# AIS-Bonn/stillleben

Measured on AMD Instinct MI355X. Metric: scenes/sec (settle + 640x480 6-ch GT render), 20-obj YCB-like, higher is better.
Workload: dtype f32; 1 GPU; C2: 20 of 21 procedural YCB-like objects (8k verts/16k tris, 1024^2 texture each) per scene; per step and GPU 32768 scenes are staged (random stack), settled (100 frames x 4 substeps), framed (camera, light, shadow matrix) and rendered at 640x480 (rgb, coord+depth, class, instance, normals; shadows on, SSAO on) -- all four stages inside the timed region; render_chunk=512, objects=20, settle_streams=1, render_streams=2, pair_contact_budget=0, parallelism=1 GPU

## Files before the change

### stillleben_amd/csrc/slhip_render.hip

```cpp
#include <algorithm>
#include <cmath>
#include <cstring>
#include <vector>
#include <type_traits>
#include "slhip_common.h"
#include "slhip_cubemap.h"
#include "slhip_raster_walk.h"

#ifndef SLHIP_RENDER_WAVES
#define SLHIP_RENDER_WAVES 0
#endif
#ifndef SLHIP_SHADE_WAVES
#define SLHIP_SHADE_WAVES 0
#endif
#ifndef SLHIP_SSAO_WAVES
#define SLHIP_SSAO_WAVES 0
#endif
#if SLHIP_RENDER_WAVES > 0
#define SLHIP_LIGHT_KERNEL __attribute__((amdgpu_waves_per_eu(1, SLHIP_RENDER_WAVES)))
#else
#define SLHIP_LIGHT_KERNEL
#endif
#if SLHIP_RENDER_WAVES > 0
#define SLHIP_SHADOW_RASTER_KERNEL SLHIP_LIGHT_KERNEL
#else
#define SLHIP_SHADOW_RASTER_KERNEL __attribute__((amdgpu_waves_per_eu(6)))
#endif
#if SLHIP_SSAO_WAVES > 0
#define SLHIP_SSAO_KERNEL __attribute__((amdgpu_waves_per_eu(1, SLHIP_SSAO_WAVES)))
#else
#define SLHIP_SSAO_KERNEL
#endif
#if SLHIP_SHADE_WAVES > 0
#define SLHIP_SHADE_KERNEL __attribute__((amdgpu_waves_per_eu(1, SLHIP_SHADE_WAVES)))
#else
#define SLHIP_SHADE_KERNEL
#endif
namespace {

static_assert(sizeof(slhip_draw) == 432, "slhip_draw layout");
static_assert(sizeof(slhip_scene) == 480, "slhip_scene layout");
static_assert(sizeof(slhip_chunk) == 16, "slhip_chunk layout");

constexpr float kInvalid = 3000.0f;
constexpr float kPi = 3.141592653589793f;
constexpr unsigned long long kVisEmpty = ~0ull;
constexpr int kSmallArea = 256;

__device__ __forceinline__ float dot3(const float* a, const float* b)
{
    float d = a[0] * b[0];
    d = fmaf(a[1], b[1], d);
    d = fmaf(a[2], b[2], d);
    return d;
}

__device__ __forceinline__ void mv4(const float* __restrict__ M, const float* v, float* o)
{
#pragma unroll
    for (int r = 0; r < 4; ++r) {
// ... 540 lines not shown
            float b[3];
#pragma unroll
            for (int k = 0; k < 3; ++k)
                b[k] = fmaf(bs[2], bary[6 + k], fmaf(bs[1], bary[3 + k], bs[0] * bary[k]));
            if (peel) {
                const float cz = interp(b, camz[0], camz[1], camz[2]);
                if (cz - 0.00001f <= peel[4 * ((size_t)py * W + px) + 3]) return;
            }
            if (pool_tex) {
                const float u = interp(b, uv[0], uv[2], uv[4]);
                const float v = interp(b, uv[1], uv[3], uv[5]);
                float bx[3], by[3];
                bary_at(t, bary, bary + 3, bary + 6, px + 1, py, bx);
                bary_at(t, bary, bary + 3, bary + 6, px, py + 1, by);
                float tc[4];
                tex_sample(pool_tex, tex, tex_w, tex_h, tex_sampler, u, v, interp(bx, uv[0], uv[2], uv[4]) - u, interp(bx, uv[1], uv[3], uv[5]) - v,
                           interp(by, uv[0], uv[2], uv[4]) - u, interp(by, uv[1], uv[3], uv[5]) - v, tc);
                if (base_alpha * tc[3] < alpha_cutoff) return;
            }
        }
        atomicMin(slot, key);
    }
};

#ifndef SLHIP_SHADOW_WINDOW
#define SLHIP_SHADOW_WINDOW 64
#endif
#ifndef SLHIP_SHADOW_WINDOW_PITCH
#define SLHIP_SHADOW_WINDOW_PITCH SLHIP_SHADOW_WINDOW
#endif
struct ShadowTarget {
    unsigned* sm;
    int W;
    unsigned* win;
    int wx0, wy0;
    unsigned wnx, wny;
    __device__ __forceinline__ void emit(const Setup& t, int px, int py, const float* l) const
    {
        const float z = interp(l, t.z[0], t.z[1], t.z[2]);
        if (!(z >= 0.0f && z <= 1.0f)) return;
        const unsigned bits = __float_as_uint(z);
#if SLHIP_SHADOW_WINDOW
        const unsigned ux = (unsigned)(px - wx0), uy = (unsigned)(py - wy0);
        if (ux < wnx && uy < wny) {
            atomicMin(win + uy * SLHIP_SHADOW_WINDOW_PITCH + ux, bits);
            return;
        }
#endif
        unsigned* slot = sm + (size_t)py * W + px;
        atomicMin(slot, bits);
    }
};

struct QItem {
    unsigned draw;
    unsigned tri_sub;
    unsigned scene_aux;
    unsigned tile;
};

template <class I, class Target>
__device__ __forceinline__ void raster_bbox_as(const Setup& t, const Target& tgt)
{
    slhip_raster::Walk<I> w;
    w.start(t.X, t.Y, t.flipped, t.bias, t.xmin, t.ymin);
    const float fa = (float)(I)t.area2;
    const int bw = t.xmax - t.xmin + 1, n = bw * (t.ymax - t.ymin + 1);
    int px = t.xmin, py = t.ymin;
    for (int k = 0; k < n; ++k) {
        if (w.inside()) {
            float l[3];
            l[0] = (float)w.numerator(0) / fa;
            l[1] = (float)w.numerator(1) / fa;
            l[2] = (float)w.numerator(2) / fa;
            tgt.emit(t, px, py, l);
        }
        if (px == t.xmax) {
            px = t.xmin; ++py;
            w.next_row();
        } else {
            ++px;
            w.step_x();
        }
    }
}

template <class Target>
__device__ __forceinline__ void raster_bbox(const Setup& t, const Target& tgt, int wide)
{
    if (!wide && __all(t.narrow)) {
        raster_bbox_as<int>(t, tgt);
    } else {
        const int bw = t.xmax - t.xmin + 1, n = bw * (t.ymax - t.ymin + 1);
        int px = t.xmin, py = t.ymin;
        for (int k = 0; k < n; ++k) {
            float l[3];
            if (coverage_as<long long>(t, px, py, l)) tgt.emit(t, px, py, l);
            if (px == t.xmax) { px = t.xmin; ++py; } else ++px;
        }
    }
}

template <class Target>
__device__ __forceinline__ void raster_or_enqueue(const Setup& t, const Target& tgt, unsigned* queue,
                                                  unsigned capacity, unsigned draw, unsigned tri_sub,
                                                  unsigned scene_aux, int small_area, int wide = 0)
{
    const int bw = t.xmax - t.xmin + 1, bh = t.ymax - t.ymin + 1;
    bool in_place = bw * bh <= small_area;
    if (!in_place) {
        const int tx0 = t.xmin >> 3, tx1 = t.xmax >> 3, ty0 = t.ymin >> 3, ty1 = t.ymax >> 3;
        const unsigned n = (unsigned)((tx1 - tx0 + 1) * (ty1 - ty0 + 1));
        const unsigned base = atomicAdd(queue, n);
        if (base + n <= capacity) {
            QItem* items = reinterpret_cast<QItem*>(queue + 4);
            unsigned k = base;
            for (int ty = ty0; ty <= ty1; ++ty)
                for (int tx = tx0; tx <= tx1; ++tx) {
                    QItem it;
                    it.draw = draw; it.tri_sub = tri_sub; it.scene_aux = scene_aux;
                    it.tile = (unsigned)tx | ((unsigned)ty << 16);
                    items[k++] = it;
                }
        } else {
            QItem* items = reinterpret_cast<QItem*>(queue + 4);
            for (unsigned k = base; k < min(base + n, capacity); ++k) {
                QItem it;
                it.draw = 0xFFFFFFFFu; it.tri_sub = 0; it.scene_aux = 0; it.tile = 0;
                items[k] = it;
            }
            in_place = true;
        }
    }
    if (in_place) raster_bbox(t, tgt, wide);
}

template <bool kAttr>
__device__ __forceinline__ void raster_chunk(unsigned chunk, const slhip_mesh_pool& pool, const slhip_scene* __restrict__ scenes,
                                             const slhip_draw* __restrict__ draws,
                                             const slhip_chunk* __restrict__ chunks, int W, int H,
                                             const float* __restrict__ depth_peel,
                                             unsigned long long* __restrict__ vis, unsigned* queue,
                                             unsigned capacity, const float4* __restrict__ clipbuf,
                                             const uint4* __restrict__ screen, int small_area, int wide)
{
    const slhip_chunk ch = chunks[chunk];
    if (threadIdx.x >= ch.count) return;
    const slhip_scene* sc = scenes + ch.scene;
    const slhip_draw* dr = draws + ch.draw;
    const bool alpha_test = (dr->flags & SLHIP_DRAW_ALPHA_TEST) && (dr->flags & SLHIP_DRAW_HAS_BASE_TEX);
    if ((alpha_test || depth_peel != nullptr) != kAttr) return;
    const unsigned tri = ch.first_tri + threadIdx.x;
    const unsigned* ip = pool.d_idx + dr->idx_base + 3 * (size_t)tri;
    const unsigned vi[3] = {ip[0], ip[1], ip[2]};
    const size_t P = (size_t)W * H;
    MainTarget tgt;
    tgt.vis = vis + (size_t)ch.scene * P;
    tgt.W = W;
    tgt.prim = dr->prim_base + tri;
    tgt.need_attr = kAttr;
    tgt.peel = nullptr;
    tgt.pool_tex = nullptr;

    if constexpr (!kAttr) {
        tgt.camz = nullptr; tgt.uv = nullptr; tgt.bary = nullptr;
        const uint4 s0 = screen[dr->clip_base + vi[0]], s1 = screen[dr->clip_base + vi[1]], s2 = screen[dr->clip_base + vi[2]];
        if (screen_all_inside(s0, s1, s2)) {
            Setup t;
            if (setup_from_screen(s0, s1, s2, W, H, t)) raster_or_enqueue(t, tgt, queue, capacity, ch.draw, tri, ch.scene, small_area, wide);
            return;
        }
        ClipVert cv[3];
#pragma unroll
        for (int k = 0; k < 3; ++k) {
            const float4 c4 = clipbuf[dr->clip_base + vi[k]];
            cv[k].clip[0] = c4.x; cv[k].clip[1] = c4.y; cv[k].clip[2] = c4.z; cv[k].clip[3] = c4.w;
            cv[k].bary[0] = cv[k].bary[1] = cv[k].bary[2] = 0.0f;
        }
        ClipVert poly[4];
        const int n = clip_near(cv, poly);
#pragma unroll
        for (int sub = 0; sub < 2; ++sub) {
            if (sub >= n - 2) break;
            Setup t;
            if (!setup_tri(poly[0].clip, poly[sub + 1].clip, poly[sub + 2].clip, W, H, t)) continue;
// ... 24 lines not shown
            for (int k = 0; k < 3; ++k) {
                const float2 uv = reinterpret_cast<const float2*>(pool.d_uv)[dr->vtx_base + vi[k]];
                uvs[2 * k] = uv.x; uvs[2 * k + 1] = uv.y;
            }
            tgt.pool_tex = pool.d_tex; tgt.tex = dr->tex_offset;
            tgt.tex_w = (int)dr->tex_w; tgt.tex_h = (int)dr->tex_h;
            tgt.tex_sampler = dr->tex_sampler[0];
        }
        tgt.camz = camz;
        tgt.uv = uvs;
        tgt.base_alpha = dr->base_color[3];
        tgt.alpha_cutoff = dr->alpha_cutoff;
#pragma unroll
        for (int sub = 0; sub < 2; ++sub) {
            if (sub >= n - 2) break;
            Setup t;
            if (!setup_tri(poly[0].clip, poly[sub + 1].clip, poly[sub + 2].clip, W, H, t)) continue;
            float bary[9];
#pragma unroll
            for (int k = 0; k < 3; ++k) {
                bary[k] = poly[0].bary[k];
                bary[3 + k] = poly[sub + 1].bary[k];
                bary[6 + k] = poly[sub + 2].bary[k];
            }
            tgt.bary = bary;
            for (int py = t.ymin; py <= t.ymax; ++py)
                for (int px = t.xmin; px <= t.xmax; ++px) {
                    float l[3];
                    if (coverage(t, px, py, l)) tgt.emit(t, px, py, l);
                }
        }
    }
}

template <bool kAttr>
__global__ __launch_bounds__(256) SLHIP_LIGHT_KERNEL void k_raster(slhip_mesh_pool pool, const slhip_scene* __restrict__ scenes,
                                                const slhip_draw* __restrict__ draws,
                                                const slhip_chunk* __restrict__ chunks, unsigned n_chunks, int W, int H,
                                                const float* __restrict__ depth_peel,
                                                unsigned long long* __restrict__ vis, unsigned* queue,
                                                unsigned capacity, const float4* __restrict__ clipbuf,
                                                const uint4* __restrict__ screen, int small_area, int wide)
{
    for (unsigned c = blockIdx.x; c < n_chunks; c += gridDim.x)
        raster_chunk<kAttr>(c, pool, scenes, draws, chunks, W, H, depth_peel, vis, queue, capacity, clipbuf, screen, small_area, wide);
}

__global__ __launch_bounds__(256) SLHIP_LIGHT_KERNEL void k_large(slhip_mesh_pool pool, const slhip_scene* __restrict__ scenes,
                                               const slhip_draw* __restrict__ draws, int W, int H,
                                               unsigned long long* __restrict__ vis,
                                               const unsigned* __restrict__ queue, unsigned capacity,
                                               const float4* __restrict__ clipbuf, const uint4* __restrict__ screen)
{
    const unsigned count = min(queue[0], capacity);
    const QItem* items = reinterpret_cast<const QItem*>(queue + 4);
    const unsigned lane = threadIdx.x & 63;
    const unsigned wave = (blockIdx.x * blockDim.x + threadIdx.x) >> 6;
    const unsigned n_waves = (gridDim.x * blockDim.x) >> 6;
    const unsigned per = (count + n_waves - 1) / n_waves;
    const unsigned i0 = wave * per, i1 = min(i0 + per, count);
    unsigned p_draw = 0xFFFFFFFFu, p_tri = 0u, p_scene = 0u, prim = 0u;
    bool ok = false;
    Setup t;
    for (unsigned i = i0; i < i1; ++i) {
        const QItem it = items[i];
        if (it.draw == 0xFFFFFFFFu) continue;
        if (it.draw != p_draw || it.tri_sub != p_tri || it.scene_aux != p_scene) {
            p_draw = it.draw; p_tri = it.tri_sub; p_scene = it.scene_aux;
            ok = false;
            const slhip_draw* dr = draws + it.draw;
            const unsigned tri = it.tri_sub & 0x7FFFFFFFu;
            const int sub = (int)(it.tri_sub >> 31);
            const unsigned* ip = pool.d_idx + dr->idx_base + 3 * (size_t)tri;
            ClipVert cv[3];
            const uint4 s0 = screen[dr->clip_base + ip[0]], s1 = screen[dr->clip_base + ip[1]], s2 = screen[dr->clip_base + ip[2]];
            const bool cached = screen_all_inside(s0, s1, s2);
            if (cached && (sub != 0 || !setup_from_screen(s0, s1, s2, W, H, t))) continue;
            if (!cached) {
#pragma unroll
                for (int k = 0; k < 3; ++k) {
                    const float4 c4 = clipbuf[dr->clip_base + ip[k]];
                    cv[k].clip[0] = c4.x; cv[k].clip[1] = c4.y; cv[k].clip[2] = c4.z; cv[k].clip[3] = c4.w;
                    cv[k].bary[0] = cv[k].bary[1] = cv[k].bary[2] = 0.0f;
                }
                ClipVert poly[4];
                const int n = clip_near(cv, poly);
                if (sub > n - 3) continue;
                const ClipVert& pb = sub == 0 ? poly[1] : poly[2];
                const ClipVert& pc = sub == 0 ? poly[2] : poly[3];
                if (!setup_tri(poly[0].clip, pb.clip, pc.clip, W, H, t)) continue;
            }
            prim = dr->prim_base + tri;
            ok = true;
        }
        if (!ok) continue;
        const int px = (int)((it.tile & 0xFFFFu) << 3) + (int)(lane & 7);
        const int py = (int)((it.tile >> 16) << 3) + (int)(lane >> 3);
        if (px < t.xmin || px > t.xmax || py < t.ymin || py > t.ymax) continue;
        float l[3];
        if (!coverage(t, px, py, l)) continue;
        MainTarget tgt;
        tgt.vis = vis + (size_t)it.scene_aux * W * H;
        tgt.peel = nullptr;
        tgt.W = W;
        tgt.prim = prim;
        tgt.need_attr = false;
        tgt.pool_tex = nullptr;
        tgt.emit(t, px, py, l);
    }
}

__device__ __forceinline__ void shadow_clip(const slhip_mesh_pool& pool, const float* T, unsigned v, float* clip)
{
    const float4 p = reinterpret_cast<const float4*>(pool.d_pos)[v];
    const float pos[4] = {p.x, p.y, p.z, 1.0f};
#pragma unroll
    for (int r = 0; r < 4; ++r) {
        float a = fmaf(T[4 * r + 0], pos[0], 0.0f);
        a = fmaf(T[4 * r + 1], pos[1], a);
        a = fmaf(T[4 * r + 2], pos[2], a);
        a = fmaf(T[4 * r + 3], pos[3], a);
        clip[r] = a;
    }
}

template <bool kMax>
__device__ __forceinline__ int wave_minmax(int v)
{
    constexpr int ident = kMax ? (int)0x80000000 : 0x7fffffff;
#define SLHIP_DPP_STEP(ctrl, rows)                                                       \
    {                                                                                    \
        const int o = __builtin_amdgcn_update_dpp(ident, v, ctrl, rows, 0xf, false);     \
        v = kMax ? max(v, o) : min(v, o);                                                \
    }
    SLHIP_DPP_STEP(0x111, 0xf) SLHIP_DPP_STEP(0x112, 0xf) SLHIP_DPP_STEP(0x114, 0xf) SLHIP_DPP_STEP(0x118, 0xf)
    SLHIP_DPP_STEP(0x142, 0xa) SLHIP_DPP_STEP(0x143, 0xc)
#undef SLHIP_DPP_STEP
    return __builtin_amdgcn_readlane(v, 63);
}

constexpr int kShadowTile = 64;
constexpr int kShadowMaxWords = 32;
__host__ __device__ inline int shadow_tiles_x(int S) { return (S + kShadowTile - 1) / kShadowTile; }
__host__ __device__ inline int shadow_tile_words(int S) { return (shadow_tiles_x(S) * shadow_tiles_x(S) + 31) / 32; }

__global__ __launch_bounds__(256) SLHIP_SHADOW_RASTER_KERNEL void k_shadow_raster(slhip_mesh_pool pool, const slhip_scene* __restrict__ scenes,
                                                       const slhip_draw* __restrict__ draws,
                                                       const slhip_chunk* __restrict__ chunks, int S,
                                                       unsigned* __restrict__ shadow, unsigned* queue,
                                                       unsigned capacity, const float4* __restrict__ clipbuf,
                                                       unsigned n_clip_verts, unsigned* __restrict__ tile_bits, int nl,
                                                       int small_area, int wide)
{
    __shared__ unsigned bm[SLHIP_NUM_LIGHTS][kShadowMaxWords];
    const slhip_chunk ch = chunks[blockIdx.x];
    if (ch.count == 0) return;
    const slhip_scene* sc = scenes + ch.scene;
    const slhip_draw* dr = draws + ch.draw;
    if (!(dr->flags & SLHIP_DRAW_CASTS_SHADOW)) return;
    const int tx_n = shadow_tiles_x(S), words = shadow_tile_words(S);
    for (int k = (int)threadIdx.x; k < SLHIP_NUM_LIGHTS * kShadowMaxWords; k += 256) bm[k / kShadowMaxWords][k % kShadowMaxWords] = 0u;
// ... 63 lines not shown
            unsigned* sm = shadow + ((size_t)ch.scene * nl + light) * S * S;
            const unsigned n = wny << wsh, cmask = (1u << wsh) - 1u;
            for (unsigned k = threadIdx.x; k < n; k += 256) {
                const unsigned v = win[(k >> wsh) * kPitch + (k & cmask)];
                const int x = wx0 + (int)(k & cmask), y = wy0 + (int)(k >> wsh);
                if (v != 0x3F800000u && x < S && y < S) atomicMin(sm + (size_t)y * S + x, v);
            }
            __syncthreads();
        }
#endif
    }
    __syncthreads();
    for (int k = (int)threadIdx.x; k < SLHIP_NUM_LIGHTS * words; k += 256) {
        const int light = k / words, w = k % words;
        if (light >= nl || !light_active(sc, light)) continue;
        const unsigned m = words <= kShadowMaxWords ? bm[light][w] : 0xFFFFFFFFu;
        if (m) atomicOr(tile_bits + ((size_t)ch.scene * SLHIP_NUM_LIGHTS + light) * words + w, m);
    }
}

__global__ __launch_bounds__(256) void k_shadow_restore(unsigned* __restrict__ shadow, unsigned* __restrict__ tile_bits, int S,
                                                        unsigned n_words_total, int nl)
{
    const unsigned wi = blockIdx.x;
    if (wi >= n_words_total) return;
    unsigned m = tile_bits[wi];
    if (m == 0u) return;
    const int words = shadow_tile_words(S), tx_n = shadow_tiles_x(S);
    const unsigned map = wi / (unsigned)words, w = wi % (unsigned)words;
    const unsigned m_scene = map / SLHIP_NUM_LIGHTS, m_light = map % SLHIP_NUM_LIGHTS;
    if ((int)m_light >= nl) return;
    unsigned* base = shadow + ((size_t)m_scene * nl + m_light) * S * S;
    const uint4 one = make_uint4(0x3F800000u, 0x3F800000u, 0x3F800000u, 0x3F800000u);
    while (m) {
        const int b = __ffs((int)m) - 1;
        m &= m - 1;
        const int tile = (int)w * 32 + b;
        const int x0 = (tile % tx_n) * kShadowTile, y0 = (tile / tx_n) * kShadowTile;
        for (int k = (int)threadIdx.x; k < kShadowTile * (kShadowTile / 4); k += 256) {
            const int y = y0 + k / (kShadowTile / 4), x = x0 + 4 * (k % (kShadowTile / 4));
            if (y < S && x < S) *reinterpret_cast<uint4*>(base + (size_t)y * S + x) = one;
        }
    }
    __syncthreads();
    if (threadIdx.x == 0) tile_bits[wi] = 0u;
}

__global__ __launch_bounds__(256) SLHIP_LIGHT_KERNEL void k_shadow_large(slhip_mesh_pool pool, const slhip_scene* __restrict__ scenes,
                                                      const slhip_draw* __restrict__ draws, int S,
                                                      unsigned* __restrict__ shadow,
                                                      const unsigned* __restrict__ queue, unsigned capacity,
                                                      const float4* __restrict__ clipbuf, unsigned n_clip_verts, int nl, int wide)
{
    const unsigned count = min(queue[0], capacity);
    const QItem* items = reinterpret_cast<const QItem*>(queue + 4);
    const unsigned lane = threadIdx.x & 63;
    const unsigned wave = (blockIdx.x * blockDim.x + threadIdx.x) >> 6;
    const unsigned n_waves = (gridDim.x * blockDim.x) >> 6;
    const unsigned per = (count + n_waves - 1) / n_waves;
    const unsigned i0 = wave * per, i1 = min(i0 + per, count);
    unsigned p_draw = 0xFFFFFFFFu, p_tri = 0u, p_scene = 0u;
    bool ok = false;
    Setup t;
    for (unsigned i = i0; i < i1; ++i) {
        const QItem it = items[i];
        if (it.draw == 0xFFFFFFFFu) continue;
        const unsigned scene = it.scene_aux & 0xFFFFFFu;
        const int light = (int)(it.scene_aux >> 24);
        if (it.draw != p_draw || it.tri_sub != p_tri || it.scene_aux != p_scene) {
            p_draw = it.draw; p_tri = it.tri_sub; p_scene = it.scene_aux;
            ok = false;
            const slhip_draw* dr = draws + it.draw;
            const unsigned* ip = pool.d_idx + dr->idx_base + 3 * (size_t)it.tri_sub;
            const float4* plane = clipbuf + (size_t)(1 + light) * n_clip_verts + dr->clip_base;
            const uint4* sp = reinterpret_cast<const uint4*>(plane);
            if (!setup_from_screen(sp[ip[0]], sp[ip[1]], sp[ip[2]], S, S, t)) continue;
            ok = true;
        }
        if (!ok) continue;
        const int px = (int)((it.tile & 0xFFFFu) << 3) + (int)(lane & 7);
        const int py = (int)((it.tile >> 16) << 3) + (int)(lane >> 3);
        if (px < t.xmin || px > t.xmax || py < t.ymin || py > t.ymax) continue;
        float l[3];
        if (!coverage_walk(t, px, py, l, wide)) continue;
        ShadowTarget tgt;
        tgt.win = nullptr; tgt.wx0 = 0; tgt.wy0 = 0; tgt.wnx = 0u; tgt.wny = 0u;
        tgt.sm = shadow + ((size_t)scene * nl + light) * S * S;
        tgt.W = S;
        tgt.emit(t, px, py, l);
    }
}

__device__ __forceinline__ float frcp(float x) { return __builtin_amdgcn_rcpf(x); }
__device__ __forceinline__ void normalize3_fast(float* v)
{
    const float r = __builtin_amdgcn_rsqf(fmaf(v[2], v[2], fmaf(v[1], v[1], v[0] * v[0])));
    v[0] *= r; v[1] *= r; v[2] *= r;
}

__device__ __forceinline__ float distribution_ggx(const float* N, const float* Hv, float roughness)
{
    const float a = roughness * roughness;
    const float a2 = a * a;
    const float NdotH = fmaxf(dot3(N, Hv), 0.0f);
    const float NdotH2 = NdotH * NdotH;
    float denom = (NdotH2 * (a2 - 1.0f) + 1.0f);
    denom = kPi * denom * denom;
    return a2 * frcp(denom);
}

__device__ __forceinline__ float geometry_schlick_ggx(float NdotV, float roughness)
{
    const float r = roughness + 1.0f;
    const float k = (r * r) * 0.125f;
    return NdotV * frcp(NdotV * (1.0f - k) + k);
}

__device__ __forceinline__ float shadow_tap(const float* __restrict__ sm, int S, float u, float v, float ref)
{
    const float x = fmaf(u, (float)S, -0.5f), y = fmaf(v, (float)S, -0.5f);
    const float fx = floorf(x), fy = floorf(y);
    const float ax = x - fx, ay = y - fy;
    int x0 = (int)fx, y0 = (int)fy, x1 = x0 + 1, y1 = y0 + 1;
    x0 = min(max(x0, 0), S - 1); x1 = min(max(x1, 0), S - 1);
    y0 = min(max(y0, 0), S - 1); y1 = min(max(y1, 0), S - 1);
    const float r = clampf(ref, 0.0f, 1.0f);
    const float c00 = r <= sm[(size_t)y0 * S + x0] ? 1.0f : 0.0f;
    const float c10 = r <= sm[(size_t)y0 * S + x1] ? 1.0f : 0.0f;
    const float c01 = r <= sm[(size_t)y1 * S + x0] ? 1.0f : 0.0f;
    const float c11 = r <= sm[(size_t)y1 * S + x1] ? 1.0f : 0.0f;
    const float top = fmaf(ax, c10 - c00, c00), bot = fmaf(ax, c11 - c01, c01);
    return fmaf(ay, bot - top, top);
}

__device__ __forceinline__ float shadow_pcf16(const float* __restrict__ sm, int S, float px, float py, float ref,
                                              const unsigned* __restrict__ tile_bits)
{
    const float scale = 1.0f / (float)S;
    int ix[4], iy[4];
    float ax[4], ay[4];
    bool regular = true;
#pragma unroll
// ... 1314 lines not shown
```

### stillleben_amd/csrc/slhip_render_stats.inc

```

namespace {

constexpr int kOsLdsSlots = 256;
constexpr int kOsLdsDraws = 256;

struct OsRec {
    unsigned px_visib, px_all;
    int bbox_visib[4], bbox_obj[4];
};
static_assert(sizeof(OsRec) == sizeof(slhip_object_stats), "slhip_object_stats layout");

__device__ __forceinline__ unsigned os_slot(const slhip_draw* dr) { return dr->instance_index & 0xFFFFu; }

__device__ __forceinline__ unsigned long long& os_word_offset(OsRec* r) { return *reinterpret_cast<unsigned long long*>(r->bbox_visib); }

__global__ __launch_bounds__(256) void k_os_init(OsRec* __restrict__ out, size_t n)
{
    for (size_t i = (size_t)blockIdx.x * blockDim.x + threadIdx.x; i < n; i += (size_t)gridDim.x * blockDim.x) {
        OsRec r;
        r.px_visib = 0u; r.px_all = 0u;
        r.bbox_visib[0] = r.bbox_visib[1] = r.bbox_visib[2] = r.bbox_visib[3] = 0;
        r.bbox_obj[0] = r.bbox_obj[1] = INT_MAX;
        r.bbox_obj[2] = r.bbox_obj[3] = INT_MIN;
        out[i] = r;
// ... 197 lines not shown
            ClipVert cv[3];
#pragma unroll
            for (int k = 0; k < 3; ++k) {
                const float4 c4 = clipbuf[dr->clip_base + vi[k]];
                cv[k].clip[0] = c4.x; cv[k].clip[1] = c4.y; cv[k].clip[2] = c4.z; cv[k].clip[3] = c4.w;
                cv[k].bary[0] = k == 0 ? 1.0f : 0.0f;
                cv[k].bary[1] = k == 1 ? 1.0f : 0.0f;
                cv[k].bary[2] = k == 2 ? 1.0f : 0.0f;
            }
            ClipVert poly[4];
            const int n = clip_near(cv, poly);
            if (n == 0) continue;
            float uvs[6];
#pragma unroll
            for (int k = 0; k < 3; ++k) {
                const float2 uv = reinterpret_cast<const float2*>(pool.d_uv)[dr->vtx_base + vi[k]];
                uvs[2 * k] = uv.x; uvs[2 * k + 1] = uv.y;
            }
            tgt.pool_tex = pool.d_tex; tgt.tex = dr->tex_offset;
            tgt.tex_w = (int)dr->tex_w; tgt.tex_h = (int)dr->tex_h;
            tgt.tex_sampler = dr->tex_sampler[0];
            tgt.uv = uvs;
            tgt.base_alpha = dr->base_color[3];
            tgt.alpha_cutoff = dr->alpha_cutoff;
#pragma unroll
            for (int sub = 0; sub < 2; ++sub) {
                if (sub >= n - 2) break;
                Setup t;
                if (!setup_tri(poly[0].clip, poly[sub + 1].clip, poly[sub + 2].clip, W, H, t)) continue;
                float bary[9];
#pragma unroll
                for (int k = 0; k < 3; ++k) {
                    bary[k] = poly[0].bary[k];
                    bary[3 + k] = poly[sub + 1].bary[k];
                    bary[6 + k] = poly[sub + 2].bary[k];
                }
                tgt.bary = bary;
                for (int py = t.ymin; py <= t.ymax; ++py)
                    for (int px = t.xmin; px <= t.xmax; ++px) {
                        float l[3];
                        if (coverage(t, px, py, l)) tgt.emit(t, px, py, l);
                    }
            }
        }
    }
}

__global__ __launch_bounds__(256) SLHIP_LIGHT_KERNEL void k_os_large(slhip_mesh_pool pool, const slhip_draw* __restrict__ draws, int W, int H,
                                                  const OsRec* __restrict__ out, unsigned n_slots,
                                                  unsigned long long* __restrict__ pool_words,
                                                  const unsigned* __restrict__ queue, unsigned capacity,
                                                  const float4* __restrict__ clipbuf, const uint4* __restrict__ screen)
{
    const unsigned count = min(queue[0], capacity);
    const QItem* items = reinterpret_cast<const QItem*>(queue + 4);
    const unsigned lane = threadIdx.x & 63;
    const unsigned wave = (blockIdx.x * blockDim.x + threadIdx.x) >> 6;
    const unsigned n_waves = (gridDim.x * blockDim.x) >> 6;
    const unsigned per = (count + n_waves - 1) / n_waves;
    const unsigned i0 = wave * per, i1 = min(i0 + per, count);
    unsigned p_draw = 0xFFFFFFFFu, p_tri = 0u, p_scene = 0u;
    bool ok = false;
    Setup t;
    StatsTarget tgt;
    for (unsigned i = i0; i < i1; ++i) {
        const QItem it = items[i];
        if (it.draw == 0xFFFFFFFFu) continue;
        if (it.draw != p_draw || it.tri_sub != p_tri || it.scene_aux != p_scene) {
            p_draw = it.draw; p_tri = it.tri_sub; p_scene = it.scene_aux;
            ok = false;
            const slhip_draw* dr = draws + it.draw;
            if (!os_target(out, n_slots, it.scene_aux, dr, pool_words, tgt)) continue;
            const unsigned tri = it.tri_sub & 0x7FFFFFFFu;
            const int sub = (int)(it.tri_sub >> 31);
            const unsigned* ip = pool.d_idx + dr->idx_base + 3 * (size_t)tri;
            const uint4 s0 = screen[dr->clip_base + ip[0]], s1 = screen[dr->clip_base + ip[1]], s2 = screen[dr->clip_base + ip[2]];
            const bool cached = screen_all_inside(s0, s1, s2);
            if (cached && (sub != 0 || !setup_from_screen(s0, s1, s2, W, H, t))) continue;
            if (!cached) {
                ClipVert cv[3];
#pragma unroll
                for (int k = 0; k < 3; ++k) {
                    const float4 c4 = clipbuf[dr->clip_base + ip[k]];
                    cv[k].clip[0] = c4.x; cv[k].clip[1] = c4.y; cv[k].clip[2] = c4.z; cv[k].clip[3] = c4.w;
                    cv[k].bary[0] = cv[k].bary[1] = cv[k].bary[2] = 0.0f;
                }
                ClipVert poly[4];
                const int n = clip_near(cv, poly);
                if (sub > n - 3) continue;
                const ClipVert& pb = sub == 0 ? poly[1] : poly[2];
                const ClipVert& pc = sub == 0 ? poly[2] : poly[3];
                if (!setup_tri(poly[0].clip, pb.clip, pc.clip, W, H, t)) continue;
            }
            ok = true;
        }
        if (!ok) continue;
        const int px = (int)((it.tile & 0xFFFFu) << 3) + (int)(lane & 7);
        const int py = (int)((it.tile >> 16) << 3) + (int)(lane >> 3);
        bool cov = !(px < t.xmin || px > t.xmax || py < t.ymin || py > t.ymax);
        float l[3];
        cov = cov && coverage(t, px, py, l);
        cov = cov && tgt.passes(t, px, py, l);
        const unsigned long long bits = __ballot(cov);
        if (lane == 0 && bits != 0ull) {
            unsigned long long* w = tgt.word(px, py);
            if (w) atomicOr(w, bits);
        }
    }
}

__global__ __launch_bounds__(256) void k_os_silhouette(OsRec* __restrict__ out, size_t n, const unsigned long long* __restrict__ pool_words)
{
    __shared__ int s_red[5][4];
    const unsigned lane = threadIdx.x & 63u, wave = threadIdx.x >> 6;
    for (size_t i = blockIdx.x; i < n; i += gridDim.x) {
        const OsRec r = out[i];
        const int tx0 = r.bbox_obj[0], ty0 = r.bbox_obj[1], tx1 = r.bbox_obj[2], ty1 = r.bbox_obj[3];
        const int tw = tx1 - tx0 + 1;
        const size_t nw = tx0 <= tx1 ? (size_t)tw * (size_t)(ty1 - ty0 + 1) : 0;
        const unsigned long long* w = pool_words + *reinterpret_cast<const unsigned long long*>(r.bbox_visib);
        int cnt = 0, xmn = INT_MAX, ymn = INT_MAX, xmx = -1, ymx = -1;
        for (size_t k = threadIdx.x; k < nw; k += blockDim.x) {
            const unsigned long long b = w[k];
            if (b == 0ull) continue;
            cnt += __popcll(b);
            unsigned cols = 0u, rows = 0u;
#pragma unroll
            for (int y = 0; y < 8; ++y) {
                const unsigned row = (unsigned)(b >> (8 * y)) & 0xFFu;
                cols |= row;
                rows |= (row != 0u ? 1u : 0u) << y;
            }
            const int tx = tx0 + (int)(k % (size_t)tw), ty = ty0 + (int)(k / (size_t)tw);
            xmn = min(xmn, tx * 8 + __ffs(cols) - 1); xmx = max(xmx, tx * 8 + 31 - __clz(cols));
            ymn = min(ymn, ty * 8 + __ffs(rows) - 1); ymx = max(ymx, ty * 8 + 31 - __clz(rows));
        }
#pragma unroll
        for (int o = 32; o > 0; o >>= 1) cnt += __shfl_xor(cnt, o);
        xmn = wave_min(xmn); ymn = wave_min(ymn); xmx = wave_max(xmx); ymx = wave_max(ymx);
        if (lane == 0u) { s_red[0][wave] = cnt; s_red[1][wave] = xmn; s_red[2][wave] = ymn; s_red[3][wave] = xmx; s_red[4][wave] = ymx; }
        __syncthreads();
        if (threadIdx.x == 0) {
            const int nwv = (int)(blockDim.x >> 6);
            for (int v = 1; v < nwv; ++v) {
                s_red[0][0] += s_red[0][v];
                s_red[1][0] = min(s_red[1][0], s_red[1][v]); s_red[2][0] = min(s_red[2][0], s_red[2][v]);
                s_red[3][0] = max(s_red[3][0], s_red[3][v]); s_red[4][0] = max(s_red[4][0], s_red[4][v]);
            }
            OsRec o;
            o.px_all = (unsigned)s_red[0][0];
            if (s_red[0][0] > 0) {
                o.bbox_obj[0] = s_red[1][0]; o.bbox_obj[1] = s_red[2][0];
                o.bbox_obj[2] = s_red[3][0] - s_red[1][0] + 1; o.bbox_obj[3] = s_red[4][0] - s_red[2][0] + 1;
            } else {
                o.bbox_obj[0] = o.bbox_obj[1] = o.bbox_obj[2] = o.bbox_obj[3] = -1;
            }
            o.px_visib = 0u;
            o.bbox_visib[0] = o.bbox_visib[1] = INT_MAX;
            o.bbox_visib[2] = o.bbox_visib[3] = -1;
// ... 196 lines not shown
```

Before: 10450 scenes/s.

## Replace per-tile raster queue items with per-triangle entries and prefix-sum tile ranges

```diff
diff --git a/stillleben_amd/csrc/slhip_render.hip b/stillleben_amd/csrc/slhip_render.hip
--- a/stillleben_amd/csrc/slhip_render.hip
+++ b/stillleben_amd/csrc/slhip_render.hip
@@ -6,6 +6,7 @@
 #include "slhip_common.h"
 #include "slhip_cubemap.h"
 #include "slhip_raster_walk.h"
+#include "slhip_tile_queue.h"
 
 #ifndef SLHIP_RENDER_WAVES
 #define SLHIP_RENDER_WAVES 0
@@ -652,11 +653,33 @@
     }
 };
 
-struct QItem {
-    unsigned draw;
-    unsigned tri_sub;
-    unsigned scene_aux;
-    unsigned tile;
+struct QueueShare {
+    const slhip_tq::Entry* entries;
+    slhip_tq::Walk walk;
+    __device__ __forceinline__ QueueShare(const unsigned* __restrict__ queue, unsigned capacity)
+    {
+        const unsigned wave = (unsigned)__builtin_amdgcn_readfirstlane((int)((blockIdx.x * blockDim.x + threadIdx.x) >> 6));
+        const unsigned n_waves = (gridDim.x * blockDim.x) >> 6;
+        entries = reinterpret_cast<const slhip_tq::Entry*>(queue + slhip_tq::kHeaderWords);
+        walk.first(slhip_tq::plan_of(queue[0], queue[1], queue[2], capacity), entries, n_waves, wave);
+    }
+};
+
+struct TilePixels {
+    unsigned ntx, tx, ty;
+    int px0, py0;
+    __device__ __forceinline__ TilePixels(const slhip_tq::Entry& en, unsigned k0, unsigned lane)
+    {
+        ntx = slhip_tq::ntx(en);
+        ty = k0 / ntx; tx = k0 - ty * ntx;
+        px0 = (int)((en.t0 & 0xFFFFu) << 3) + (int)(lane & 7);
+        py0 = (int)((en.t0 >> 16) << 3) + (int)(lane >> 3);
+    }
+    __device__ __forceinline__ void next(int& px, int& py)
+    {
+        px = px0 + (int)(tx << 3); py = py0 + (int)(ty << 3);
+        if (++tx == ntx) { tx = 0u; ++ty; }
+    }
 };
 
 template <class I, class Target>
@@ -709,28 +732,18 @@
     const int bw = t.xmax - t.xmin + 1, bh = t.ymax - t.ymin + 1;
     bool in_place = bw * bh <= small_area;
     if (!in_place) {
-        const int tx0 = t.xmin >> 3, tx1 = t.xmax >> 3, ty0 = t.ymin >> 3, ty1 = t.ymax >> 3;
-        const unsigned n = (unsigned)((tx1 - tx0 + 1) * (ty1 - ty0 + 1));
-        const unsigned base = atomicAdd(queue, n);
-        if (base + n <= capacity) {
-            QItem* items = reinterpret_cast<QItem*>(queue + 4);
-            unsigned k = base;
-            for (int ty = ty0; ty <= ty1; ++ty)
-                for (int tx = tx0; tx <= tx1; ++tx) {
-                    QItem it;
-                    it.draw = draw; it.tri_sub = tri_sub; it.scene_aux = scene_aux;
-                    it.tile = (unsigned)tx | ((unsigned)ty << 16);
-                    items[k++] = it;
-                }
-        } else {
-            QItem* items = reinterpret_cast<QItem*>(queue + 4);
-            for (unsigned k = base; k < min(base + n, capacity); ++k) {
-                QItem it;
-                it.draw = 0xFFFFFFFFu; it.tri_sub = 0; it.scene_aux = 0; it.tile = 0;
-                items[k] = it;
-            }
-            in_place = true;
-        }
+        const unsigned tx0 = (unsigned)(t.xmin >> 3), ty0 = (unsigned)(t.ymin >> 3);
+        const unsigned ntx = (unsigned)(t.xmax >> 3) - tx0 + 1u, nty = (unsigned)(t.ymax >> 3) - ty0 + 1u;
+        const unsigned n = ntx * nty;
+        const slhip_tq::Slot s =
+            slhip_tq::slot_of(atomicAdd(reinterpret_cast<unsigned long long*>(queue), slhip_tq::reservation(n)), n, capacity);
+        if (s.carried) atomicOr(queue + 2, 1u);
+        if (s.fits) {
+            uint4* e = reinterpret_cast<uint4*>(queue + slhip_tq::kHeaderWords) + slhip_tq::kUnitsPerEntry * (size_t)s.index;
+            e[0] = make_uint4(draw, tri_sub, scene_aux, s.tile_base);
+            e[1] = make_uint4(tx0 | (ty0 << 16), s.carried ? 0u : (ntx | (nty << 16)), 0u, 0u);
+        }
+        in_place = !s.fits || s.carried;
     }
     if (in_place) raster_bbox(t, tgt, wide);
 }
@@ -861,61 +874,52 @@
                                                const unsigned* __restrict__ queue, unsigned capacity,
                                                const float4* __restrict__ clipbuf, const uint4* __restrict__ screen)
 {
-    const unsigned count = min(queue[0], capacity);
-    const QItem* items = reinterpret_cast<const QItem*>(queue + 4);
+    const QueueShare q(queue, capacity);
     const unsigned lane = threadIdx.x & 63;
-    const unsigned wave = (blockIdx.x * blockDim.x + threadIdx.x) >> 6;
-    const unsigned n_waves = (gridDim.x * blockDim.x) >> 6;
-    const unsigned per = (count + n_waves - 1) / n_waves;
-    const unsigned i0 = wave * per, i1 = min(i0 + per, count);
-    unsigned p_draw = 0xFFFFFFFFu, p_tri = 0u, p_scene = 0u, prim = 0u;
-    bool ok = false;
-    Setup t;
-    for (unsigned i = i0; i < i1; ++i) {
-        const QItem it = items[i];
-        if (it.draw == 0xFFFFFFFFu) continue;
-        if (it.draw != p_draw || it.tri_sub != p_tri || it.scene_aux != p_scene) {
-            p_draw = it.draw; p_tri = it.tri_sub; p_scene = it.scene_aux;
-            ok = false;
-            const slhip_draw* dr = draws + it.draw;
-            const unsigned tri = it.tri_sub & 0x7FFFFFFFu;
-            const int sub = (int)(it.tri_sub >> 31);
-            const unsigned* ip = pool.d_idx + dr->idx_base + 3 * (size_t)tri;
-            ClipVert cv[3];
-            const uint4 s0 = screen[dr->clip_base + ip[0]], s1 = screen[dr->clip_base + ip[1]], s2 = screen[dr->clip_base + ip[2]];
-            const bool cached = screen_all_inside(s0, s1, s2);
-            if (cached && (sub != 0 || !setup_from_screen(s0, s1, s2, W, H, t))) continue;
-            if (!cached) {
-#pragma unroll
-                for (int k = 0; k < 3; ++k) {
-                    const float4 c4 = clipbuf[dr->clip_base + ip[k]];
-                    cv[k].clip[0] = c4.x; cv[k].clip[1] = c4.y; cv[k].clip[2] = c4.z; cv[k].clip[3] = c4.w;
-                    cv[k].bary[0] = cv[k].bary[1] = cv[k].bary[2] = 0.0f;
-                }
-                ClipVert poly[4];
-                const int n = clip_near(cv, poly);
-                if (sub > n - 3) continue;
-                const ClipVert& pb = sub == 0 ? poly[1] : poly[2];
-                const ClipVert& pc = sub == 0 ? poly[2] : poly[3];
-                if (!setup_tri(poly[0].clip, pb.clip, pc.clip, W, H, t)) continue;
+    for (unsigned e = q.walk.e0; e < q.walk.e1; ++e) {
+        const slhip_tq::Entry en = q.entries[e];
+        if (q.walk.done(en)) break;
+        unsigned k0, k1;
+        if (!q.walk.tiles(en, k0, k1)) continue;
+        Setup t;
+        const slhip_draw* dr = draws + en.draw;
+        const unsigned tri = en.tri_sub & 0x7FFFFFFFu;
+        const int sub = (int)(en.tri_sub >> 31);
+        const unsigned* ip = pool.d_idx + dr->idx_base + 3 * (size_t)tri;
+        ClipVert cv[3];
+        const uint4 s0 = screen[dr->clip_base + ip[0]], s1 = screen[dr->clip_base + ip[1]], s2 = screen[dr->clip_base + ip[2]];
+        const bool cached = screen_all_inside(s0, s1, s2);
+        if (cached && (sub != 0 || !setup_from_screen(s0, s1, s2, W, H, t))) continue;
+        if (!cached) {
+#pragma unroll
+            for (int k = 0; k < 3; ++k) {
+                const float4 c4 = clipbuf[dr->clip_base + ip[k]];
+                cv[k].clip[0] = c4.x; cv[k].clip[1] = c4.y; cv[k].clip[2] = c4.z; cv[k].clip[3] = c4.w;
+                cv[k].bary[0] = cv[k].bary[1] = cv[k].bary[2] = 0.0f;
             }
-            prim = dr->prim_base + tri;
-            ok = true;
-        }
-        if (!ok) continue;
-        const int px = (int)((it.tile & 0xFFFFu) << 3) + (int)(lane & 7);
-        const int py = (int)((it.tile >> 16) << 3) + (int)(lane >> 3);
-        if (px < t.xmin || px > t.xmax || py < t.ymin || py > t.ymax) continue;
-        float l[3];
-        if (!coverage(t, px, py, l)) continue;
+            ClipVert poly[4];
+            const int n = clip_near(cv, poly);
+            if (sub > n - 3) continue;
+            const ClipVert& pb = sub == 0 ? poly[1] : poly[2];
+            const ClipVert& pc = sub == 0 ? poly[2] : poly[3];
+            if (!setup_tri(poly[0].clip, pb.clip, pc.clip, W, H, t)) continue;
+        }
         MainTarget tgt;
-        tgt.vis = vis + (size_t)it.scene_aux * W * H;
+        tgt.vis = vis + (size_t)en.scene_aux * W * H;
         tgt.peel = nullptr;
         tgt.W = W;
-        tgt.prim = prim;
+        tgt.prim = dr->prim_base + tri;
         tgt.need_attr = false;
         tgt.pool_tex = nullptr;
-        tgt.emit(t, px, py, l);
+        TilePixels tp(en, k0, lane);
+        for (unsigned k = k0; k < k1; ++k) {
+            int px, py;
+            tp.next(px, py);
+            if (px < t.xmin || px > t.xmax || py < t.ymin || py > t.ymax) continue;
+            float l[3];
+            if (!coverage(t, px, py, l)) continue;
+            tgt.emit(t, px, py, l);
+        }
     }
 }
 
@@ -1085,42 +1089,34 @@
                                                       const unsigned* __restrict__ queue, unsigned capacity,
                                                       const float4* __restrict__ clipbuf, unsigned n_clip_verts, int nl, int wide)
 {
-    const unsigned count = min(queue[0], capacity);
-    const QItem* items = reinterpret_cast<const QItem*>(queue + 4);
+    const QueueShare q(queue, capacity);
     const unsigned lane = threadIdx.x & 63;
-    const unsigned wave = (blockIdx.x * blockDim.x + threadIdx.x) >> 6;
-    const unsigned n_waves = (gridDim.x * blockDim.x) >> 6;
-    const unsigned per = (count + n_waves - 1) / n_waves;
-    const unsigned i0 = wave * per, i1 = min(i0 + per, count);
-    unsigned p_draw = 0xFFFFFFFFu, p_tri = 0u, p_scene = 0u;
-    bool ok = false;
-    Setup t;
-    for (unsigned i = i0; i < i1; ++i) {
-        const QItem it = items[i];
-        if (it.draw == 0xFFFFFFFFu) continue;
-        const unsigned scene = it.scene_aux & 0xFFFFFFu;
-        const int light = (int)(it.scene_aux >> 24);
-        if (it.draw != p_draw || it.tri_sub != p_tri || it.scene_aux != p_scene) {
-            p_draw = it.draw; p_tri = it.tri_sub; p_scene = it.scene_aux;
-            ok = false;
-            const slhip_draw* dr = draws + it.draw;
-            const unsigned* ip = pool.d_idx + dr->idx_base + 3 * (size_t)it.tri_sub;
-            const float4* plane = clipbuf + (size_t)(1 + light) * n_clip_verts + dr->clip_base;
-            const uint4* sp = reinterpret_cast<const uint4*>(plane);
-            if (!setup_from_screen(sp[ip[0]], sp[ip[1]], sp[ip[2]], S, S, t)) continue;
-            ok = true;
-        }
-        if (!ok) continue;
-        const int px = (int)((it.tile & 0xFFFFu) << 3) + (int)(lane & 7);
-        const int py = (int)((it.tile >> 16) << 3) + (int)(lane >> 3);
-        if (px < t.xmin || px > t.xmax || py < t.ymin || py > t.ymax) continue;
-        float l[3];
-        if (!coverage_walk(t, px, py, l, wide)) continue;
+    for (unsigned e = q.walk.e0; e < q.walk.e1; ++e) {
+        const slhip_tq::Entry en = q.entries[e];
+        if (q.walk.done(en)) break;
+        unsigned k0, k1;
+        if (!q.walk.tiles(en, k0, k1)) continue;
+        const unsigned scene = en.scene_aux & 0xFFFFFFu;
+        const int light = (int)(en.scene_aux >> 24);
+        Setup t;
+        const slhip_draw* dr = draws + en.draw;
+        const unsigned* ip = pool.d_idx + dr->idx_base + 3 * (size_t)en.tri_sub;
+        const float4* plane = clipbuf + (size_t)(1 + light) * n_clip_verts + dr->clip_base;
+        const uint4* sp = reinterpret_cast<const uint4*>(plane);
+        if (!setup_from_screen(sp[ip[0]], sp[ip[1]], sp[ip[2]], S, S, t)) continue;
         ShadowTarget tgt;
         tgt.win = nullptr; tgt.wx0 = 0; tgt.wy0 = 0; tgt.wnx = 0u; tgt.wny = 0u;
         tgt.sm = shadow + ((size_t)scene * nl + light) * S * S;
         tgt.W = S;
-        tgt.emit(t, px, py, l);
+        TilePixels tp(en, k0, lane);
+        for (unsigned k = k0; k < k1; ++k) {
+            int px, py;
+            tp.next(px, py);
+            if (px < t.xmin || px > t.xmax || py < t.ymin || py > t.ymax) continue;
+            float l[3];
+            if (!coverage_walk(t, px, py, l, wide)) continue;
+            tgt.emit(t, px, py, l);
+        }
     }
 }
 
diff --git a/stillleben_amd/csrc/slhip_render_stats.inc b/stillleben_amd/csrc/slhip_render_stats.inc
--- a/stillleben_amd/csrc/slhip_render_stats.inc
+++ b/stillleben_amd/csrc/slhip_render_stats.inc
@@ -273,59 +273,51 @@
                                                   const unsigned* __restrict__ queue, unsigned capacity,
                                                   const float4* __restrict__ clipbuf, const uint4* __restrict__ screen)
 {
-    const unsigned count = min(queue[0], capacity);
-    const QItem* items = reinterpret_cast<const QItem*>(queue + 4);
+    const QueueShare q(queue, capacity);
     const unsigned lane = threadIdx.x & 63;
-    const unsigned wave = (blockIdx.x * blockDim.x + threadIdx.x) >> 6;
-    const unsigned n_waves = (gridDim.x * blockDim.x) >> 6;
-    const unsigned per = (count + n_waves - 1) / n_waves;
-    const unsigned i0 = wave * per, i1 = min(i0 + per, count);
-    unsigned p_draw = 0xFFFFFFFFu, p_tri = 0u, p_scene = 0u;
-    bool ok = false;
-    Setup t;
-    StatsTarget tgt;
-    for (unsigned i = i0; i < i1; ++i) {
-        const QItem it = items[i];
-        if (it.draw == 0xFFFFFFFFu) continue;
-        if (it.draw != p_draw || it.tri_sub != p_tri || it.scene_aux != p_scene) {
-            p_draw = it.draw; p_tri = it.tri_sub; p_scene = it.scene_aux;
-            ok = false;
-            const slhip_draw* dr = draws + it.draw;
-            if (!os_target(out, n_slots, it.scene_aux, dr, pool_words, tgt)) continue;
-            const unsigned tri = it.tri_sub & 0x7FFFFFFFu;
-            const int sub = (int)(it.tri_sub >> 31);
-            const unsigned* ip = pool.d_idx + dr->idx_base + 3 * (size_t)tri;
-            const uint4 s0 = screen[dr->clip_base + ip[0]], s1 = screen[dr->clip_base + ip[1]], s2 = screen[dr->clip_base + ip[2]];
-            const bool cached = screen_all_inside(s0, s1, s2);
-            if (cached && (sub != 0 || !setup_from_screen(s0, s1, s2, W, H, t))) continue;
-            if (!cached) {
-                ClipVert cv[3];
-#pragma unroll
-                for (int k = 0; k < 3; ++k) {
-                    const float4 c4 = clipbuf[dr->clip_base + ip[k]];
-                    cv[k].clip[0] = c4.x; cv[k].clip[1] = c4.y; cv[k].clip[2] = c4.z; cv[k].clip[3] = c4.w;
-                    cv[k].bary[0] = cv[k].bary[1] = cv[k].bary[2] = 0.0f;
-                }
-                ClipVert poly[4];
-                const int n = clip_near(cv, poly);
-                if (sub > n - 3) continue;
-                const ClipVert& pb = sub == 0 ? poly[1] : poly[2];
-                const ClipVert& pc = sub == 0 ? poly[2] : poly[3];
-                if (!setup_tri(poly[0].clip, pb.clip, pc.clip, W, H, t)) continue;
-            }
-            ok = true;
-        }
-        if (!ok) continue;
-        const int px = (int)((it.tile & 0xFFFFu) << 3) + (int)(lane & 7);
-        const int py = (int)((it.tile >> 16) << 3) + (int)(lane >> 3);
-        bool cov = !(px < t.xmin || px > t.xmax || py < t.ymin || py > t.ymax);
-        float l[3];
-        cov = cov && coverage(t, px, py, l);
-        cov = cov && tgt.passes(t, px, py, l);
-        const unsigned long long bits = __ballot(cov);
-        if (lane == 0 && bits != 0ull) {
-            unsigned long long* w = tgt.word(px, py);
-            if (w) atomicOr(w, bits);
+    for (unsigned e = q.walk.e0; e < q.walk.e1; ++e) {
+        const slhip_tq::Entry en = q.entries[e];
+        if (q.walk.done(en)) break;
+        unsigned k0, k1;
+        if (!q.walk.tiles(en, k0, k1)) continue;
+        Setup t;
+        StatsTarget tgt;
+        const slhip_draw* dr = draws + en.draw;
+        if (!os_target(out, n_slots, en.scene_aux, dr, pool_words, tgt)) continue;
+        const unsigned tri = en.tri_sub & 0x7FFFFFFFu;
+        const int sub = (int)(en.tri_sub >> 31);
+        const unsigned* ip = pool.d_idx + dr->idx_base + 3 * (size_t)tri;
+        const uint4 s0 = screen[dr->clip_base + ip[0]], s1 = screen[dr->clip_base + ip[1]], s2 = screen[dr->clip_base + ip[2]];
+        const bool cached = screen_all_inside(s0, s1, s2);
+        if (cached && (sub != 0 || !setup_from_screen(s0, s1, s2, W, H, t))) continue;
+        if (!cached) {
+            ClipVert cv[3];
+#pragma unroll
+            for (int k = 0; k < 3; ++k) {
+                const float4 c4 = clipbuf[dr->clip_base + ip[k]];
+                cv[k].clip[0] = c4.x; cv[k].clip[1] = c4.y; cv[k].clip[2] = c4.z; cv[k].clip[3] = c4.w;
+                cv[k].bary[0] = cv[k].bary[1] = cv[k].bary[2] = 0.0f;
+            }
+            ClipVert poly[4];
+            const int n = clip_near(cv, poly);
+            if (sub > n - 3) continue;
+            const ClipVert& pb = sub == 0 ? poly[1] : poly[2];
+            const ClipVert& pc = sub == 0 ? poly[2] : poly[3];
+            if (!setup_tri(poly[0].clip, pb.clip, pc.clip, W, H, t)) continue;
+        }
+        TilePixels tp(en, k0, lane);
+        for (unsigned k = k0; k < k1; ++k) {
+            int px, py;
+            tp.next(px, py);
+            bool cov = !(px < t.xmin || px > t.xmax || py < t.ymin || py > t.ymax);
+            float l[3];
+            cov = cov && coverage(t, px, py, l);
+            cov = cov && tgt.passes(t, px, py, l);
+            const unsigned long long bits = __ballot(cov);
+            if (lane == 0 && bits != 0ull) {
+                unsigned long long* w = tgt.word(px, py);
+                if (w) atomicOr(w, bits);
+            }
         }
     }
 }
diff --git a/stillleben_amd/csrc/slhip_tile_queue.h b/stillleben_amd/csrc/slhip_tile_queue.h
--- /dev/null
+++ b/stillleben_amd/csrc/slhip_tile_queue.h
@@ -0,0 +1,114 @@
+#pragma once
+
+#include <stdint.h>
+
+#if defined(__HIPCC__)
+#define SLHIP_TQ_HD __host__ __device__ __forceinline__
+#else
+#define SLHIP_TQ_HD inline
+#endif
+
+namespace slhip_tq {
+
+constexpr unsigned kHeaderWords = 4;
+constexpr unsigned kUnitsPerEntry = 2;
+
+struct Entry {
+    unsigned draw;
+    unsigned tri_sub;
+    unsigned scene_aux;
+    unsigned tile_base;
+    unsigned t0;
+    unsigned nt;
+    unsigned spare[2];
+};
+static_assert(sizeof(Entry) == 16 * kUnitsPerEntry, "an entry is two 16-byte units");
+
+SLHIP_TQ_HD unsigned entry_capacity(unsigned capacity_units) { return capacity_units / kUnitsPerEntry; }
+SLHIP_TQ_HD unsigned ntx(const Entry& e) { return e.nt & 0xFFFFu; }
+SLHIP_TQ_HD unsigned nty(const Entry& e) { return e.nt >> 16; }
+SLHIP_TQ_HD unsigned n_tiles(const Entry& e) { return ntx(e) * nty(e); }
+
+SLHIP_TQ_HD unsigned long long reservation(unsigned n) { return 1ull | ((unsigned long long)n << 32); }
+
+struct Slot {
+    unsigned index;
+    unsigned tile_base;
+    bool fits;
+    bool carried;
+};
+SLHIP_TQ_HD Slot slot_of(unsigned long long before, unsigned n, unsigned capacity_units)
+{
+    Slot s;
+    s.index = (unsigned)before;
+    s.tile_base = (unsigned)(before >> 32);
+    s.fits = s.index < entry_capacity(capacity_units);
+    s.carried = (unsigned long long)s.tile_base + n > 0xFFFFFFFFull;
+    return s;
+}
+
+struct Plan {
+    unsigned count;
+    unsigned total;
+    bool by_entries;
+};
+SLHIP_TQ_HD Plan plan_of(unsigned entries, unsigned tiles, unsigned carried, unsigned capacity_units)
+{
+    Plan p;
+    const unsigned cap = entry_capacity(capacity_units);
+    p.count = entries < cap ? entries : cap;
+    p.by_entries = carried != 0u;
+    p.total = p.by_entries ? p.count : tiles;
+    if (p.count == 0u) p.total = 0u;
+    return p;
+}
+
+SLHIP_TQ_HD void range_of(unsigned total, unsigned n_ranges, unsigned r, unsigned& t0, unsigned& t1)
+{
+    const unsigned long long per = ((unsigned long long)total + n_ranges - 1) / n_ranges;
+    const unsigned long long a = per * r, b = a + per;
+    t0 = (unsigned)(a < total ? a : total);
+    t1 = (unsigned)(b < total ? b : total);
+}
+
+SLHIP_TQ_HD unsigned find_entry(const Entry* entries, unsigned count, unsigned t)
+{
+    unsigned lo = 0, hi = count;
+    while (hi - lo > 1u) {
+        const unsigned mid = lo + (hi - lo) / 2;
+        if (entries[mid].tile_base <= t) lo = mid; else hi = mid;
+    }
+    return lo;
+}
+
+struct Walk {
+    unsigned t0, t1;
+    unsigned e0, e1;
+    bool by_entries;
+
+    SLHIP_TQ_HD void first(const Plan& p, const Entry* entries, unsigned n_ranges, unsigned r)
+    {
+        by_entries = p.by_entries;
+        unsigned a, b;
+        range_of(p.total, n_ranges, r, a, b);
+        if (by_entries) {
+            e0 = a; e1 = b; t0 = 0u; t1 = 0xFFFFFFFFu;
+        } else {
+            t0 = a; t1 = b; e1 = p.count;
+            e0 = a < b ? find_entry(entries, p.count, a) : p.count;
+        }
+    }
+    SLHIP_TQ_HD bool done(const Entry& e) const { return !by_entries && e.tile_base >= t1; }
+    SLHIP_TQ_HD bool tiles(const Entry& e, unsigned& k0, unsigned& k1) const
+    {
+        const unsigned n = n_tiles(e);
+        if (by_entries) { k0 = 0u; k1 = n; return n != 0u; }
+        const unsigned base = e.tile_base, end = base + n;
+        const unsigned lo = t0 > base ? t0 : base, hi = t1 < end ? t1 : end;
+        if (lo >= hi) return false;
+        k0 = lo - base; k1 = hi - base;
+        return true;
+    }
+};
+
+}
```

New measurement: 10640 scenes/s, median of 6. 1.8% higher.
